# SahakyanLab/GenomeAssembler_dev

Measured on AMD Instinct MI355X. Metric: k-mers built+scored/sec, higher is better.
Workload: dtype u64 keys / u32 counts / f64 scores; 1 GPU; cfg2 (configs[2]): 100 x 50000 bp segments per GPU, 150 bp reads at 50x, k=31, build + breakage scoring of all contigs; mode=segments, segments_total=100, distinct_kmers_rank0=3843627, parallelism=segments sharded over 1 GPU(s), no collective

## Files before the change

### genomeassembler_dev_amd/csrc/kernels.h

```cpp
#pragma once
#include <hip/hip_runtime.h>
#include <stdint.h>

#include "device_utils.h"
#include "keyops.h"

struct ReadSet {
    const u64* words;
    const u64* read_off;
    const u64* seg_read_off;
    const u32* seg_tile_start;
    const uint4* tile_info;
    u32 fixed_len;
    u32 n_segments;
};

__device__ __forceinline__ void read_span(const ReadSet& rs, u64 r, u64* p0, u32* len) {
    if (rs.fixed_len) { *p0 = rs.read_off ? rs.read_off[r] : r * rs.fixed_len; *len = rs.fixed_len; }
    else { const u64 a = rs.read_off[r]; *p0 = a; *len = (u32)(rs.read_off[r + 1] - a); }
}

struct GraphView {
    const void* dk_key;
    const u32* dstart;
// ... 131 lines not shown
template <class K>
__global__ void k_tip_mark(GraphView gv, u32 n_segments, u32 chunks, const u8* eflag, const u32* clen, const u32* nxt, const u32* dk_cnt, const u64* bstart,
                           u32* mult, u32 tip_len, u32* flags, u32* tips);
template <class K>
__global__ void k_bubble_mark(GraphView gv, u32 n_segments, u32 chunks, const u8* eflag, const u32* clen, const u32* nxt, const u32* dk_cnt, const u64* bstart,
                              u32* mult, u32 bubble_len, u32* flags, u32* bubbles);
__global__ void k_kmer_spectrum(const u32* dstart, u32 nb, const u32* dk_cnt, u32 n_segments, u32 chunks, u32* hist);
template <class K>
__global__ void k_lowcov_mark(GraphView gv, u32 n_segments, u32 chunks, const u8* eflag, const u32* clen, const u32* nxt, const u32* dk_cnt, const u64* bstart,
                              u32* mult, u32 cov_len, u32 cov_cutoff, u32* flags, u32* removed);
__global__ void k_contig_cov(const u32* dstart, u32 nb, u32 n_segments, u32 chunks, const u64* link, const u32* e_cid, const u32* dk_cnt,
                             const u32* seg_cstart, unsigned long long* msum, u32* nedges);
template <class K>
__global__ void k_bucket_gather(const K* keys, const u32* mult, const u64* bstart, const u32* dstart, K* dk_key, u32* dk_cnt, u32* claim, u8* eflag,
                                u32* flags);
template <class K> __global__ void k_edge_target(GraphView gv, u32 n_segments, u32 chunks, u32* tgt, u32* claim);
__global__ void k_edge_multi(GraphView gv, u32 n_segments, u32 chunks, const u32* tgt, const u32* claim, u8* eflag);
template <class K>
__global__ void k_node_flags(GraphView gv, u32 n_segments, u32 chunks, const u32* claim, u8* eflag, u64* link, u32* clen);
__global__ void k_edge_next(GraphView gv, u32 n_segments, u32 chunks, const u32* tgt, const u8* eflag, u32* nxt, u64* link);
__global__ void k_link_jump(GraphView gv, u32 n_segments, u32 chunks, u64* link, const u32* prev_active, u32* active, int jumps, const u32* nxt,
                            u32* clen);
__global__ void k_rank_rulers(GraphView gv, u32 n_segments, u32 chunks, u64* link, u32* rtab, u32 rshift, u32* flags);
__global__ void k_rank_lds(GraphView gv, const u32* rtab, u64* link, int max_rounds, u32 rshift, u32 lds_entries, u32* flags);
__global__ void k_chain_len(const u32* nxt, const u64* link, u32* clen, const u32* n_edges_p);
__global__ void k_contig_scan(GraphView gv, const u8* eflag, const u32* clen, u32* e_cid, u64* e_coff, u32* seg_ncontig,
                              u64* seg_cbases, u32* done, u32* seg_cstart, u64* seg_bstart, const u32* flags, u32* report, u32 ticket);
__global__ void k_contig_place(GraphView gv, const u8* eflag, const u32* seg_cstart, const u64* seg_bstart, u32* e_cid, u64* e_coff,
                               u64* c_off, u32 n_segments, u32 chunks);
template <class K>
__global__ void k_contig_emit(GraphView gv, const u64* link, const u32* nxt, const u64* e_coff, u8* out, u32 n_segments, u32 chunks);
__global__ void k_reads_both_strands(const u64* words, const u64* read_off, const u64* seg_read_off, u32 fixed_len, u32 n_segments, u64 n_reads, u32 g,
                                     unsigned long long* out);
template <class K>
__global__ void k_contig_twin(GraphView gv, const u64* link, const u32* e_cid, const u64* c_off, const u32* seg_cstart, const u8* text, u32 n_segments,
                              u32* twin, u32* bad);

template <class K>
__global__ void k_pack_runs(const K* keys, const u32* mult, const u64* bstart, const u32* bucket_d, const u32* gb_list, const u64* dst_off, K* out_keys,
                            u32* out_cnt);
template <class K, int TBL>
__global__ void k_bucket_merge(const K* in_keys, const u32* in_cnt, const u64* run_off, const u32* run_len, u32 n_src, K* out_keys, u32* out_cnt,
                               const u64* bstart, u32* bucket_d, u32* overflow, u16* fdir, int low_bits, const u64* src_base);
__global__ void k_repack_reads(const u64* src, const u64* dir, u64* words_out);
__global__ void k_piece_positions(const u64* piece_first, const u64* piece_word_off, u32 n_pieces, u64 n_reads, u32 fixed_len, u64* pos);
__global__ void k_slice_last(const u32* a, const u64* off, u32 n, u32* out);

__global__ void k_chain_expand(const u64* cwords, const u64* c_off, const u64* sig_off, const u32* elem_contig, const u32* elem_skip, const u64* elem_pos,
                               const u64* out_off, u32 n_scaffolds, u64* out, u64 n_words);
struct ChainSigs {
    const u64* sig_off;
    const u32* elem_contig;
// ... 99 lines not shown
```

### genomeassembler_dev_amd/csrc/kernels_build.hip

```cpp
#include "device_utils.h"
#include "keyops.h"
#include "kernels.h"
#include "dedup_order.h"

typedef unsigned long long u64x2 __attribute__((ext_vector_type(2)));

typedef unsigned int u32x4nt __attribute__((ext_vector_type(4)));
__device__ __forceinline__ uint4 stream_load16(const uint4* p) {
    const u32x4nt v = __builtin_nontemporal_load(reinterpret_cast<const u32x4nt*>(p));
    return make_uint4(v.x, v.y, v.z, v.w);
}
__device__ __forceinline__ void stream_store16(u64x2 v, u64x2* p) { __builtin_nontemporal_store(v, p); }

__global__ void __launch_bounds__(GASM_WG) k_pack_ascii(const u8* __restrict__ ascii, u64 nbases_host, const u64* __restrict__ nbases_dev,
                                                        u64* __restrict__ words, u32* __restrict__ err) {
    const u64 nbases = nbases_dev ? *nbases_dev : nbases_host;
    const u64 nwords = (nbases + 31) / 32 + 4;
    bool ok = true;
    for (u64 t = (u64)blockIdx.x * GASM_WG + threadIdx.x; t < nwords; t += (u64)gridDim.x * GASM_WG) {
        const u64 b0 = t << 5;
        u64 w = 0;
        if (b0 + 32 <= nbases) {
            const uint4* src = reinterpret_cast<const uint4*>(ascii + b0);
            const uint4 v0 = src[0], v1 = src[1];
// ... 123 lines not shown
        for (int d = 1; d < 64; d <<= 1) {
            const u64 o = __shfl_up(inc, d, 64);
            if ((int)ln >= d) inc += o;
        }
        if (ln == 63) s_wave[wv] = inc;
        __syncthreads();
        u64 before = 0, tot = 0;
#pragma unroll
        for (u32 w = 0; w < 16; ++w) { const u64 t = s_wave[w]; if (w < wv) before += t; tot += t; }
        __syncthreads();
        u64 ex = carry + before + inc - sum;
#pragma unroll
        for (u32 q = 0; q < 8; ++q) {
            if (i0 + q < n) out[i0 + q] = (TO)ex;
            ex += v[q];
        }
        carry += tot;
    }
    if (threadIdx.x == 0) out[n] = (TO)carry;
}
template __global__ void k_scan_excl<u64>(const u32*, u64*, u32);
template __global__ void k_scan_excl<u32>(const u32*, u32*, u32);

__device__ __forceinline__ void seg_offsets_wave(const u32* __restrict__ seg_ncontig, const u64* __restrict__ seg_cbases, u32 S,
                                                 u32* __restrict__ seg_cstart, u64* __restrict__ seg_bstart,
                                                 const u32* __restrict__ dstart, u32 nb, const u32* __restrict__ flags,
                                                 u32* __restrict__ report, u32 ticket) {
    const u32 ln = threadIdx.x & 63;
    u32 ccarry = 0;
    u64 bcarry = 0;
    const BuildReport<u32> rep{report, S};
    u32* const rc = &rep.cstart(0);
    u32* const rb = &rep.bstart_lo(0);
    for (u32 base = 0; base < S; base += 64) {
        const u32 i = base + ln;
        const u32 c = i < S ? __hip_atomic_load(&seg_ncontig[i], __ATOMIC_RELAXED, __HIP_MEMORY_SCOPE_AGENT) : 0u;
        const u64 b = i < S ? __hip_atomic_load(&seg_cbases[i], __ATOMIC_RELAXED, __HIP_MEMORY_SCOPE_AGENT) : 0ull;
        const u32 cinc = wave_incl_scan(c);
        u64 binc = b;
#pragma unroll
        for (int d = 1; d < 64; d <<= 1) {
            const u64 o = __shfl_up(binc, d, 64);
            if ((int)ln >= d) binc += o;
        }
        if (i < S) {
            const u32 cs = ccarry + cinc - c;
            const u64 bs = bcarry + binc - b;
            seg_cstart[i] = cs; seg_bstart[i] = bs;
            rc[i] = cs;
            rb[2 * i] = (u32)bs; rb[2 * i + 1] = (u32)(bs >> 32);
            rep.dstart(i) = dstart[(u64)i * nb];
        }
        ccarry += wave_last(cinc);
        bcarry += __shfl(binc, 63, 64);
    }
    if (ln == 0) {
        seg_cstart[S] = ccarry; seg_bstart[S] = bcarry;
        rc[S] = ccarry;
        rb[2 * S] = (u32)bcarry; rb[2 * S + 1] = (u32)(bcarry >> 32);
        rep.dstart(S) = dstart[(u64)S * nb];
        rep.flags() = flags[GASM_FLAG_OVERFLOW];
        rep.rank_failed() = flags[GASM_FLAG_RANK_FAILED];
    }
    __threadfence_system();
    if (ln == 0) rep.ticket() = ticket;
}

template <class K> struct TilePrefetch {
    Roll<K> rl;
    u32 nv, c01, c23, toff, bs_lo, bs_hi;
    template <int N> __device__ __forceinline__ void wait_all_but() {
        rl.template wait_all_but<N>();
        __asm__ volatile("" : "+v"(c01), "+v"(c23), "+v"(toff), "+v"(bs_lo), "+v"(bs_hi));
    }
};

template <class K>
__global__ void __launch_bounds__(GASM_TILE_WG, 1024 / GASM_TILE_WG) k_bucket_scatter(ReadSet rs, const uint4* __restrict__ tinfo, int k, int bbits, u32 g, u32 padm,
                                                                  u32 n_tiles, const u64* __restrict__ bstart, const u32* __restrict__ toff,
                                                                  const ushort4* __restrict__ tcnt, K* __restrict__ keys, u64 scratch) {
    extern __shared__ __align__(16) unsigned char s_raw[];
    constexpr u32 KT = KeyTraits<K>::KT;
    constexpr u32 NFL = KeyTraits<K>::NFL;
    constexpr u32 KPU = TileStage<K>::KPU;
    constexpr u32 CAP = TileStage<K>::CAP;
    const u32 nb = 1u << bbits;
    const u32 tid = threadIdx.x, wv = tid >> 6, ln = tid & 63, sub = tid & 3u;
    const ScatterLds<K> lds{nb};
// ... 809 lines not shown
    const u32 lo = gv.dstart[seg * nb], hi = gv.dstart[(seg + 1) * nb];
    const u32 nr = (hi - lo + rmask) >> rshift;
    for (u32 r = chunk * GASM_WG + threadIdx.x; r < nr; r += chunks * GASM_WG) {
        const u32 i = lo + (r << rshift);
        u32 cur = i, acc = 0, e = GASM_RANK_NONE;
        int step = 0;
        for (; step < 4096; ++step) {
            const u64 l = link[cur];
            if (cur != i) link[cur] = ((u64)i << 32) | GASM_LINK_TAG | acc;
            const u32 a = (u32)(l >> 32);
            if (a == GASM_NONE32) break;
            acc += (u32)l & 0x7FFFFFFFu;
            const u32 al = a - lo;
            if ((l & GASM_LINK_DONE) || !(al & rmask)) { e = (al << 16) | acc; break; }
            if (a == i) break;
            cur = a;
        }
        if (step == 4096) flags[GASM_FLAG_RANK_FAILED] = 1u;
        rtab[(lo >> rshift) + seg + r] = e;
    }
}

#define GASM_RANK_DEAD 0x8000FFFFu
__global__ void __launch_bounds__(1024) k_rank_lds(GraphView gv, const u32* __restrict__ rtab, u64* __restrict__ link, int max_rounds,
                                                    u32 rshift, u32 lds_entries, u32* __restrict__ flags) {
    const u32 rmask = (1u << rshift) - 1u;
    extern __shared__ u32 s_e[];
    __shared__ u32 s_active;
    const u32 seg = blockIdx.x;
    const u32 nb = 1u << gv.bbits;
    const u32 lo = gv.dstart[seg * nb], hi = gv.dstart[(seg + 1) * nb];
    const u32 nr = (hi - lo + rmask) >> rshift;
    if (nr > lds_entries || hi - lo > 65534u) { if (threadIdx.x == 0) flags[GASM_FLAG_RANK_FAILED] = 1u; return; }
    const u32* src = rtab + (lo >> rshift) + seg;
    u32 mine[32];
    u32 live = 0;
#pragma unroll
    for (u32 q = 0; q < 32; ++q) {
        const u32 r = threadIdx.x + 1024 * q;
        u32 e = r < nr ? src[r] : GASM_RANK_NONE;
        bool hopping = false;
        if (e == GASM_RANK_NONE) e = GASM_RANK_DEAD;
        else {
            const u32 a = e >> 16;
            if ((a & rmask) || (a == (r << rshift) && !(e & 0xFFFFu))) e = (0x8000u | r) << 16;
            else if (a == (r << rshift)) e = GASM_RANK_DEAD;
            else { e = ((a >> rshift) << 16) | (e & 0xFFFFu); hopping = true; }
        }
        mine[q] = e;
        if (r < nr) s_e[r] = e;
        live |= (u32)hopping << q;
    }
    for (int round = 0; round < max_rounds; ++round) {
        if (threadIdx.x == 0) s_active = 0;
        __syncthreads();
        u32 any = 0;
#pragma unroll
        for (u32 q0 = 0; q0 < 32; q0 += 8) {
            if (((live >> q0) & 0xFFu) == 0) continue;
            u32 x[8];
#pragma unroll
            for (u32 u = 0; u < 8; ++u) x[u] = s_e[(mine[q0 + u] >> 16) & 0x7FFFu];
#pragma unroll
            for (u32 u = 0; u < 8; ++u) {
                const u32 q = q0 + u;
                const u32 r = threadIdx.x + 1024 * q, e = mine[q];
                const u32 lv = (live >> q) & 1u, stop = x[u] >> 31;
                const u32 hop = lv & ~stop;
                const u32 hopped = (x[u] & 0xFFFF0000u) | ((e + x[u]) & 0xFFFFu);
                const u32 ne = hop ? hopped : e;
                live &= ~((lv & stop) << q);
                any |= hop;
                mine[q] = ne;
                s_e[min(r, nr)] = ne;
            }
        }
        if (any) s_active = 1;
        __syncthreads();
        const bool go = s_active != 0;
        __syncthreads();
        if (!go) break;
    }
#pragma unroll
    for (u32 q = 0; q < 32; ++q) {
        const u32 r = threadIdx.x + 1024 * q;
        if (r >= nr) continue;
        const u32 e = mine[q];
        u64 l = ~0ull;
        if (!((live >> q) & 1u) && e != GASM_RANK_DEAD) {
            const u32 t = (e >> 16) & 0x7FFFu;
            if (s_e[t] != GASM_RANK_DEAD) {
                const u32 ot = src[t];
                l = ((u64)(lo + (ot >> 16)) << 32) | GASM_LINK_DONE | (((e & 0xFFFFu) + (ot & 0xFFFFu)) & 0xFFFFu);
            }
        }
        link[lo + (r << rshift)] = l;
    }
}

__global__ void __launch_bounds__(GASM_WG) k_chain_len(const u32* __restrict__ nxt, const u64* __restrict__ link, u32* __restrict__ clen,
                                                       const u32* __restrict__ n_edges_p) {
    const u32 n_edges = *n_edges_p;
    for (u32 i = blockIdx.x * GASM_WG + threadIdx.x; i < n_edges; i += gridDim.x * GASM_WG) {
        if (nxt[i] != GASM_NONE32) continue;
        const u64 l = link[i];
        const u32 a = (u32)(l >> 32);
        if (a == GASM_NONE32 || !(l & GASM_LINK_DONE)) continue;
        clen[a] = ((u32)l & 0x7FFFFFFFu) + 1;
    }
}

__global__ void __launch_bounds__(1024) k_contig_scan(GraphView gv, const u8* __restrict__ eflag, const u32* __restrict__ clen,
                                                      u32* __restrict__ e_cid, u64* __restrict__ e_coff,
                                                      u32* __restrict__ seg_ncontig, u64* __restrict__ seg_cbases,
                                                      u32* __restrict__ done, u32* __restrict__ seg_cstart, u64* __restrict__ seg_bstart,
                                                      const u32* __restrict__ flags, u32* __restrict__ report, u32 ticket) {
    __shared__ u32 s_last;
    __shared__ u32 s_cnt[16];
    __shared__ u64 s_bas[16];
    const u32 seg = blockIdx.x;
    const u32 nb = 1u << gv.bbits;
    const u32 lo = gv.dstart[seg * nb], hi = gv.dstart[(seg + 1) * nb];
    const u32 wv = threadIdx.x >> 6, ln = threadIdx.x & 63;
    const u32 per = ((hi - lo + 15) / 16 + 63) & ~63u;
    const u32 wa = min(hi, lo + wv * per), wb = min(hi, wa + per);
    u32 ccarry = 0;
    u64 bcarry = 0;
    for (u32 base = wa; base < wb; base += 1024) {
        u32 ef[16];
        u32 cl[16];
#pragma unroll
        for (u32 q = 0; q < 16; ++q) {
            const u32 i = base + q * 64 + ln;
            ef[q] = i < wb ? (u32)eflag[i] : 0u;
            cl[q] = i < wb ? clen[i] : 0u;
        }
#pragma unroll
        for (u32 q = 0; q < 16; ++q) __asm__ volatile("" : "+v"(cl[q]), "+v"(ef[q]));
#pragma unroll
        for (u32 q = 0; q < 16; ++q) {
            const u32 i = base + q * 64 + ln;
            const bool head = ef[q] & 1;
            const u32 len = head ? (u32)(gv.k - 1) + cl[q] : 0u;
            const u32 cinc = wave_incl_scan(head ? 1u : 0u);
            const u32 binc = wave_incl_scan(len);
            if (head) { e_cid[i] = ccarry + cinc - 1; e_coff[i] = bcarry + binc - len; }
            ccarry += wave_last(cinc);
            bcarry += wave_last(binc);
        }
    }
    if (ln == 0) { s_cnt[wv] = ccarry; s_bas[wv] = bcarry; }
    __syncthreads();
    u32 cbefore = 0, ctot = 0;
    u64 bbefore = 0, btot = 0;
#pragma unroll
    for (u32 w = 0; w < 16; ++w) {
        if (w < wv) { cbefore += s_cnt[w]; bbefore += s_bas[w]; }
        ctot += s_cnt[w]; btot += s_bas[w];
    }
    if (wv) {
        for (u32 base = wa + ln; base < wb; base += 2048) {
            u32 ef[32];
#pragma unroll
            for (u32 q = 0; q < 32; ++q) ef[q] = base + 64 * q < wb ? (u32)eflag[base + 64 * q] : 0u;
#pragma unroll
            for (u32 q = 0; q < 32; ++q)
                if (ef[q] & 1) { e_cid[base + 64 * q] += cbefore; e_coff[base + 64 * q] += bbefore; }
        }
    }
    if (threadIdx.x == 0) {
        publish_u32(&seg_ncontig[seg], ctot); publish_u64(&seg_cbases[seg], btot);
        s_last = count_in_last(done) ? 1u : 0u;
    }
    __syncthreads();
    if (!s_last || wv) return;
    seg_offsets_wave(seg_ncontig, seg_cbases, gridDim.x, seg_cstart, seg_bstart, gv.dstart, nb, flags, report, ticket);
}

__global__ void __launch_bounds__(GASM_WG) k_contig_place(GraphView gv, const u8* __restrict__ eflag,
                                                          const u32* __restrict__ seg_cstart, const u64* __restrict__ seg_bstart,
                                                          u32* __restrict__ e_cid, u64* __restrict__ e_coff,
                                                          u64* __restrict__ c_off, u32 n_segments, u32 chunks) {
    if (blockIdx.x == 0 && threadIdx.x == 0) c_off[seg_cstart[n_segments]] = seg_bstart[n_segments];
    for_seg_edges(gv.dstart, 1u << gv.bbits, n_segments, chunks, [&](u32 seg, u32, u32, u32 i) {
        if (!(eflag[i] & 1)) return;
        const u32 cid = seg_cstart[seg] + e_cid[i];
        const u64 off = seg_bstart[seg] + e_coff[i];
        e_cid[i] = cid;
        e_coff[i] = off;
        c_off[cid] = off;
    });
}

__device__ __forceinline__ u32 klow16(u64 a) { return (u32)a & 0xFFFFu; }
__device__ __forceinline__ u32 klow16(const K128& a) { return (u32)a.lo & 0xFFFFu; }
template <class K>
__global__ void __launch_bounds__(GASM_WG) k_contig_emit(GraphView gv, const u64* __restrict__ link, const u32* __restrict__ nxt,
                                                         const u64* __restrict__ e_coff, u8* __restrict__ out, u32 n_segments,
                                                         u32 chunks) {
    for_seg_edge_groups(gv.dstart, 1u << gv.bbits, n_segments, chunks, [&](u32, u32, u32, const u32 (&i)[GASM_EDGE_ILP], const bool (&ok)[GASM_EDGE_ILP]) {
        u64 l[GASM_EDGE_ILP], off[GASM_EDGE_ILP];
        u32 nx[GASM_EDGE_ILP];
        K key[GASM_EDGE_ILP];
        bool on[GASM_EDGE_ILP];
        const int k = gv.k;
        const bool wide = k >= 8;
#pragma unroll
        for (int q = 0; q < GASM_EDGE_ILP; ++q) {
            l[q] = ok[q] ? link[i[q]] : ~0ull;
            nx[q] = ok[q] ? nxt[i[q]] : 0u;
// ... 288 lines not shown
```

### genomeassembler_dev_amd/csrc/pipeline.hip

```cpp
#include <atomic>
#include <chrono>
#include <thread>
#include "pipeline.h"

#include <algorithm>
#include <cmath>

__global__ void k_set_u64(u64* p, u64 v) { *p = v; }

__global__ void k_add_empty_reads(PathSet ps, const u64* __restrict__ seg_empty, u32* __restrict__ poscnt, u32* __restrict__ total) {
    const u32 seg = blockIdx.y;
    const u32 p = ps.seg_path_off[seg] + blockIdx.x * GASM_WG + threadIdx.x;
    if (p >= ps.seg_path_off[seg + 1]) return;
    const u32 e = (u32)seg_empty[seg];
    if (!e) return;
    if (ps.p_off[p + 1] > ps.p_off[p]) poscnt[ps.p_off[p]] += e;
    else total[p] += e;
}

struct Knobs {
    int dedup_tbl = 0, scatter_wgs = 8, hist_wgs = 64, rank_rounds = 18, bbits_add = 0, ruler_shift = 0;
    bool rank_global = false, sync_build = false;
    Knobs() {
        if (const char* v = getenv("GASM_DEDUP_TBL")) dedup_tbl = atoi(v);
// ... 385 lines not shown
                    &d_eflag, &d_nxt, &d_link, &d_clen, &d_ecid, &d_ecoff, &d_rtab, &d_seg_cbases, &d_seg_cstart,
                    &d_seg_bstart, &d_c_off, &d_contig_ascii})
        b->release();
    for (RoundStats& rs : round_stats) rs.d_stats.release();
    part_valid = false;
    if (h_report) { (void)hipHostFree(h_report); h_report = nullptr; h_report_words = 0; }
}

void ScoreState::release() {
    for (DBuf* b : {&d_tbl_off, &d_seed, &d_gpos, &d_poscnt, &d_total, &d_out_f64, &d_out_i32, &d_freq, &d_pd_off, &d_pd, &d_seg_empty, &d_fxsum, &d_first, &d_first_off}) b->release();
}

static int ensure_lds_attrs(gasm_ctx* ctx) {
    if (ctx->lds_attrs_set) return GASM_OK;
#define GASM_LDS_ATTR(kern, bytes) HIPCHK(hipFuncSetAttribute(reinterpret_cast<const void*>(kern), hipFuncAttributeMaxDynamicSharedMemorySize, bytes));
#define GASM_SCORE_LDS_ATTR(T) GASM_LDS_ATTR((k_score_reads_graph<K, T>), GASM_SCORE_PATH_CAP * 12)
    for (int words = 1; words <= 2; ++words)
        GCHK(with_key(words, [&](auto tag) -> int {
            using K = typename decltype(tag)::type;
            GASM_LDS_ATTR(k_bucket_scatter<K>, 160 * 1024) GASM_LDS_ATTR(k_bucket_partition<K>, 160 * 1024) GASM_LDS_ATTR(k_tile_hist<K>, 160 * 1024)
            GASM_SCORE_LDS_ATTR(1) GASM_SCORE_LDS_ATTR(2) GASM_SCORE_LDS_ATTR(3) GASM_SCORE_LDS_ATTR(4) GASM_SCORE_LDS_ATTR(5) GASM_SCORE_LDS_ATTR(6) GASM_SCORE_LDS_ATTR(7) GASM_SCORE_LDS_ATTR(8)
            return GASM_OK;
        }));
    GASM_LDS_ATTR(k_rank_lds, 160 * 1024 - 64)
#undef GASM_SCORE_LDS_ATTR
#undef GASM_LDS_ATTR
    ctx->lds_attrs_set = true;
    return GASM_OK;
}

void distinct_caps(BuildState& bs, u32 S) {
    const u64 limit = bs.multi_pass ? GASM_BUCKET_MAX : bs.small_tbl ? GASM_TBL_LIMIT / 2 : GASM_TBL_LIMIT;
    const u64 per_seg = ((u64)1 << bs.bbits) * limit;
    const u64 all = bs.k < 16 ? ((u64)1 << (2 * bs.k)) : ~(u64)0;
    bs.D_cap = 0; bs.maxD_cap = 0;
    for (u32 s = 0; s < S; ++s) {
        const u64 c = std::min(std::min(bs.h_seg_nk[s], per_seg), all);
        bs.D_cap += c;
        bs.maxD_cap = std::max(bs.maxD_cap, c);
    }
}

static int launch_graph_dense(gasm_ctx* ctx, u32 S, BuildState& bs, bool last_pass);

static GraphView graph_view(const BuildState& bs) {
    GraphView gv;
    gv.dk_key = bs.d_dk_key.p;
    gv.dstart = bs.d_dstart.as<u32>();
    gv.fdir = bs.d_fdir.as<u16>();
    gv.k = bs.k;
    gv.bbits = bs.bbits;
    gv.fbits = bs.fbits;
    return gv;
}

template <class K, int TBL>
static int launch_bucket_dedup_as(gasm_ctx* ctx, BuildState& bs, u32 nbt, const u32* d_blen, u32* d_scan_out) {
    GLAUNCH(ctx, "k_bucket_dedup", (k_bucket_dedup<K, TBL>), dim3(nbt), dim3(GASM_WG), 0, bs.d_keys.as<K>(), bs.d_mult.as<u32>(), bs.d_bstart.as<u64>(), d_blen,
            bs.d_bucket_d.as<u32>(), bs.d_flags.as<u32>(), bs.d_fdir.as<u16>(), 2 * bs.k - bs.bbits, d_scan_out);
    return GASM_OK;
}
static int launch_bucket_dedup(gasm_ctx* ctx, BuildState& bs, u32 nbt, const u32* d_blen, u32* d_scan_out) {
    if (bs.words == 2) return launch_bucket_dedup_as<K128, 2048>(ctx, bs, nbt, d_blen, d_scan_out);
    if (bs.small_tbl) return launch_bucket_dedup_as<u64, 2048>(ctx, bs, nbt, d_blen, d_scan_out);
    return launch_bucket_dedup_as<u64, 4096>(ctx, bs, nbt, d_blen, d_scan_out);
}
// ... 85 lines not shown
        GCHK(bs.d_solid_removed.ensure((size_t)S * 4));
        HIPCHK(hipMemsetAsync(bs.d_solid_removed.p, 0, (size_t)S * 4, ctx->stream));
        GLAUNCH_K(ctx, W, "k_bucket_solid", k_bucket_solid<K>, dim3(nbt), dim3(GASM_WG), 0, bs.d_keys.as<K>(), bs.d_mult.as<u32>(), bs.d_bstart.as<u64>(),
                  bs.d_bucket_d.as<u32>(), bs.d_fdir.as<u16>(), 2 * k - bbits, bs.fbits, bbits, bs.opts.min_count, bs.d_solid_removed.as<u32>(),
                  bs.d_flags.as<u32>() + GASM_FLAG_SOLID_DONE, d_scan_out);
    }
    if (!scan_in_dedup) GLAUNCH(ctx, "k_scan_excl", k_scan_excl<u32>, dim3(1), dim3(1024), 0, bs.d_bucket_d.as<u32>(), bs.d_dstart.as<u32>(), nbt);
    return GASM_OK;
}

static int alloc_graph(BuildState& bs, u32 S) {
    const u64 D = std::max<u64>(bs.D_cap, 1);
    const size_t KB = 8 * (size_t)bs.words;
    if (D >= 0xFFFFFFF0ull) { gasm_set_error("more than 2^32 distinct k-mers possible in one batch: split it"); return GASM_ERR_CAPACITY; }
    GCHK(bs.d_dk_key.ensure(D * KB));
    GCHK(bs.d_dk_cnt.ensure(D * 4));
    GCHK(bs.d_eflag.ensure(D));
    GCHK(bs.d_nxt.ensure(D * 4));
    GCHK(bs.d_link.ensure(D * 8));
    GCHK(bs.d_clen.ensure(D * 4));
    GCHK(bs.d_ecid.ensure(D * 4));
    GCHK(bs.d_ecoff.ensure(D * 8));
    GCHK(bs.d_rtab.ensure((D / 2 + S + 2) * 4));
    GCHK(bs.d_seg_cbases.ensure((size_t)S * 8 + (size_t)S * 4));
    GCHK(bs.d_seg_cstart.ensure(((size_t)S + 1) * 4));
    GCHK(bs.d_seg_bstart.ensure(((size_t)S + 1) * 8));
    bs.bases_cap = D * (u64)bs.k;
    if (bs.bases_cap >= 0xFFFFFFF0ull) { gasm_set_error("contigs could exceed 2^32 bases: split the batch"); return GASM_ERR_CAPACITY; }
    GCHK(bs.d_c_off.ensure((D + 1) * 8));
    GCHK(bs.d_contig_ascii.ensure(bs.bases_cap + 64));
    return GASM_OK;
}

int launch_graph(gasm_ctx* ctx, u32 S, BuildState& bs) {
    const int W = bs.words, bbits = bs.bbits;
    const u32 nb = 1u << bbits, nbt = S * nb;
    GCHK(alloc_graph(bs, S));
    u32* const d_claim = bs.d_nxt.as<u32>();
    const BuildOpts& o = bs.opts;
    const u32 rounds = o.total_rounds();
    for (u32 kind = 0; kind < ROUND_KINDS; ++kind) {
        RoundStats& rs = bs.round_stats[kind];
        if (!o.rounds(kind)) continue;
        GCHK(rs.d_stats.ensure((size_t)2 * rs.max_rounds * S * 4));
        HIPCHK(hipMemsetAsync(rs.d_stats.p, 0, (size_t)2 * rs.max_rounds * S * 4, ctx->stream));
    }
    for (u32 r = 0; r <= rounds; ++r) {
// ... 14 lines not shown
            GLAUNCH_K(ctx, W, "k_tip_mark", k_tip_mark<K>, seg_grid(dchunks, S), dim3(GASM_WG), 0, graph_view(bs), S, dchunks, bs.d_eflag.as<u8>(), bs.d_clen.as<u32>(),
                      bs.d_nxt.as<u32>(), bs.d_dk_cnt.as<u32>(), bs.d_bstart.as<u64>(), bs.d_mult.as<u32>(), o.tip_len, bs.d_flags.as<u32>(), d_contigs);
        } else if (kind == ROUNDS_BUBBLE) {
            GLAUNCH_K(ctx, W, "k_bubble_mark", k_bubble_mark<K>, seg_grid(dchunks, S), dim3(GASM_WG), 0, graph_view(bs), S, dchunks, bs.d_eflag.as<u8>(),
                      bs.d_clen.as<u32>(), bs.d_nxt.as<u32>(), bs.d_dk_cnt.as<u32>(), bs.d_bstart.as<u64>(), bs.d_mult.as<u32>(), o.bubble_len,
                      bs.d_flags.as<u32>(), d_contigs);
        } else {
            GLAUNCH_K(ctx, W, "k_lowcov_mark", k_lowcov_mark<K>, seg_grid(dchunks, S), dim3(GASM_WG), 0, graph_view(bs), S, dchunks, bs.d_eflag.as<u8>(),
                      bs.d_clen.as<u32>(), bs.d_nxt.as<u32>(), bs.d_dk_cnt.as<u32>(), bs.d_bstart.as<u64>(), bs.d_mult.as<u32>(), o.cov_len, o.cov_cutoff,
                      bs.d_flags.as<u32>(), d_contigs);
        }
        u32* const d_scan_out = bs.scan_in_dedup ? bs.d_dstart.as<u32>() : nullptr;
        GLAUNCH_K(ctx, W, "k_bucket_solid", k_bucket_solid<K>, dim3(nbt), dim3(GASM_WG), 0, bs.d_keys.as<K>(), bs.d_mult.as<u32>(), bs.d_bstart.as<u64>(),
                  bs.d_bucket_d.as<u32>(), bs.d_fdir.as<u16>(), 2 * bs.k - bbits, bs.fbits, bbits, 1u, d_kmers, bs.d_flags.as<u32>() + GASM_FLAG_SOLID_DONE, d_scan_out);
        if (!d_scan_out) GLAUNCH(ctx, "k_scan_excl", k_scan_excl<u32>, dim3(1), dim3(1024), 0, bs.d_bucket_d.as<u32>(), bs.d_dstart.as<u32>(), nbt);
    }
    return GASM_OK;
}

static int launch_graph_dense(gasm_ctx* ctx, u32 S, BuildState& bs, bool last_pass) {
    GasmRange range("gasm:graph (degrees, list ranking, contigs)");
    const int W = bs.words;
    u32* const d_claim = bs.d_nxt.as<u32>();
    u32* const d_seg_ncontig = reinterpret_cast<u32*>(bs.d_seg_cbases.as<u64>() + S);
    u32* const d_fl = bs.d_flags.as<u32>();
    const GraphView gv = graph_view(bs);
    const u32 nb = 1u << bs.bbits;
    const u32 est = std::max<u32>(1, (u32)std::min<u64>(bs.maxD_est, bs.maxD_cap));
    const u32 dchunks = (u32)ceil_div_u64(est, GASM_WG);
    const dim3 grid_seg = seg_grid(dchunks, S);
    const u32 gchunks = (u32)ceil_div_u64(est, GASM_WG * GASM_EDGE_ILP);
    const dim3 grid_grp = seg_grid(gchunks, S);
    u32* const d_tgt = bs.d_ecid.as<u32>();
    GLAUNCH_K(ctx, W, "k_edge_target", k_edge_target<K>, grid_seg, dim3(GASM_WG), 0, gv, S, dchunks, d_tgt, d_claim);
    GLAUNCH(ctx, "k_edge_multi", k_edge_multi, grid_grp, dim3(GASM_WG), 0, gv, S, gchunks, d_tgt, d_claim, bs.d_eflag.as<u8>());
    GLAUNCH_K(ctx, W, "k_node_flags", k_node_flags<K>, grid_seg, dim3(GASM_WG), 0, gv, S, dchunks, d_claim, bs.d_eflag.as<u8>(), bs.d_link.as<u64>(), bs.d_clen.as<u32>());
    GLAUNCH(ctx, "k_edge_next", k_edge_next, grid_grp, dim3(GASM_WG), 0, gv, S, gchunks, d_tgt, bs.d_eflag.as<u8>(), bs.d_nxt.as<u32>(), bs.d_link.as<u64>());
    u32* const act = d_fl + GASM_FLAG_ACTIVE;
    const u32 jchunks = (u32)ceil_div_u64(est, GASM_WG * GASM_JUMP_ILP);
    bs.ranked_in_lds = est <= 65534 && !bs.rank_global && !knobs().rank_global;
    bs.ruler_shift = 0;
    if (bs.ranked_in_lds) {
        const u32 rshift = knobs().ruler_shift ? (u32)knobs().ruler_shift : (S >= (u32)ctx->n_cu / 4 ? 1u : 2u);
        bs.ruler_shift = rshift;
        const u32 rchunks = (u32)ceil_div_u64((est + (1u << rshift) - 1) >> rshift, GASM_WG);
        u32 lds_entries = 32767;
        if (S > (u32)ctx->n_cu) lds_entries = std::min<u32>(32767, (((est + est / 4) >> rshift) + 1024) & ~1023u);
        GLAUNCH(ctx, "k_rank_rulers", k_rank_rulers, seg_grid(rchunks, S), dim3(GASM_WG), 0, gv, S, rchunks, bs.d_link.as<u64>(), bs.d_rtab.as<u32>(), rshift, d_fl);
        GLAUNCH(ctx, "k_rank_lds", k_rank_lds, dim3(S), dim3(1024), (size_t)lds_entries * 4 + 4, gv, bs.d_rtab.as<u32>(), bs.d_link.as<u64>(), knobs().rank_rounds, rshift,
                lds_entries, d_fl);
        const int jumps = 255, launches = 2;
        static_assert(launches <= GASM_FLAG_ACTIVE_N, "an active word per launch");
        for (int r = 0; r < launches; ++r)
            GLAUNCH(ctx, "k_link_jump", k_link_jump, seg_grid(jchunks, S), dim3(GASM_WG), 0, gv, S, jchunks, bs.d_link.as<u64>(), r ? act + r - 1 : nullptr, act + r, jumps,
                    bs.d_nxt.as<u32>(), bs.d_clen.as<u32>());
    } else {
        int rounds = 1;
        while ((1ull << rounds) < bs.maxD_cap) ++rounds;
        rounds += 1;
        const int jumps = 4, launches = (rounds * 10 + 22) / 23 + 1;
        if (launches > (int)GASM_FLAG_ACTIVE_N) { gasm_set_error("segment too large for the list-ranking flags"); return GASM_ERR_CAPACITY; }
        for (int r = 0; r < launches; ++r)
            GLAUNCH(ctx, "k_link_jump", k_link_jump, seg_grid(jchunks, S), dim3(GASM_WG), 0, gv, S, jchunks, bs.d_link.as<u64>(), r ? act + r - 1 : nullptr, act + r, jumps,
                    (const u32*)nullptr, (u32*)nullptr);
    }
    const u32 grid_all = (u32)std::min<u64>(ceil_div_u64((u64)est * S, GASM_WG), (u64)ctx->n_cu * 64);
    if (!bs.ranked_in_lds)
        GLAUNCH(ctx, "k_chain_len", k_chain_len, dim3(std::max(1u, grid_all)), dim3(GASM_WG), 0, bs.d_nxt.as<u32>(), bs.d_link.as<u64>(),
                bs.d_clen.as<u32>(), gv.dstart + (size_t)S * nb);
    if (!last_pass) return GASM_OK;
    const size_t words = BuildReport<u32>::words(S);
    if (bs.h_report_words < words) {
        if (bs.h_report) (void)hipHostFree(bs.h_report);
        bs.h_report = nullptr; bs.h_report_words = 0;
        HIPCHK(hipHostMalloc((void**)&bs.h_report, words * 4, hipHostMallocCoherent));
        bs.h_report_words = words;
    }
    bs.ticket = next_ticket();
    BuildReport<volatile u32>{bs.h_report, S}.ticket() = 0;
    GLAUNCH(ctx, "k_contig_scan", k_contig_scan, dim3(S), dim3(1024), 0, gv, bs.d_eflag.as<u8>(), bs.d_clen.as<u32>(),
            bs.d_ecid.as<u32>(), bs.d_ecoff.as<u64>(), d_seg_ncontig, bs.d_seg_cbases.as<u64>(), d_fl + GASM_FLAG_CONTIG_DONE, bs.d_seg_cstart.as<u32>(),
            bs.d_seg_bstart.as<u64>(), d_fl, bs.h_report, bs.ticket);
    GLAUNCH(ctx, "k_contig_place", k_contig_place, grid_seg, dim3(GASM_WG), 0, gv, bs.d_eflag.as<u8>(),
            bs.d_seg_cstart.as<u32>(), bs.d_seg_bstart.as<u64>(), bs.d_ecid.as<u32>(), bs.d_ecoff.as<u64>(), bs.d_c_off.as<u64>(), S, dchunks);
    GLAUNCH_K(ctx, W, "k_contig_emit", k_contig_emit<K>, grid_grp, dim3(GASM_WG), 0, gv, bs.d_link.as<u64>(), bs.d_nxt.as<u32>(),
              bs.d_ecoff.as<u64>(), bs.d_contig_ascii.as<u8>(), S, gchunks);
    bs.pending = true;
    return GASM_OK;
}

int plan_build(gasm_ctx* ctx, DevReads& rd, int k, u64 hint, BuildState& bs) {
    if (k < 2 || k > GASM_MAX_K) { gasm_set_error("k = %d not supported (2..%d)", k, GASM_MAX_K); return GASM_ERR_INVALID; }
    const int W = k <= 31 ? 1 : 2;
    const u32 KT = (u32)with_key(W, [](auto tag) -> int { return KeyTraits<typename decltype(tag)::type>::KT; });
    HIPCHK(hipSetDevice(ctx->device));
    GCHK(ensure_lds_attrs(ctx));
    const u32 S = rd.n_segments;
    const bool same = bs.k == k && bs.words == W && bs.h_seg_nk.size() == S && bs.hint == hint && bs.reads_id == rd.upload_id;
    bs.words = W; bs.k = k; bs.hint = hint; bs.reads_id = rd.upload_id;
    bs.fetched_distinct = bs.fetched_contigs = false;
    bs.pending = false;
    u64 N = 0, maxNs = 0;
    bs.h_seg_nk.assign(S, 0);
    if (rd.fixed_len) {
        const u64 nk = rd.fixed_len >= (u32)k ? rd.fixed_len - k + 1 : 0;
        for (u32 s = 0; s < S; ++s) bs.h_seg_nk[s] = (rd.h_seg_read_off[s + 1] - rd.h_seg_read_off[s]) * nk;
    } else {
// ... 1064 lines not shown
```

Measured before the change: 231.4 billion k-mers/s.

## Split contig scan into per-wave units across workgroups and shrink rank_lds workgroup

The contig prefix scan no longer runs one 1024-thread workgroup per segment. It is spread over several GASM_WG-sized workgroups per segment, each wave publishing a unit count and base sum. A block-wide scan over all units in the last workgroup replaces the per-segment wave scan, and contig_place then applies per-unit offsets, which removes the second fix-up pass over eflag. k_rank_lds moves to 512-thread groups with capped LDS and rereads its entries from LDS instead of keeping a 32-entry register array, so it can sit on a CU beside other kernels. The cost is a larger unit buffer and a serial final scan over S*units entries.

```diff
diff --git a/genomeassembler_dev_amd/csrc/kernels.h b/genomeassembler_dev_amd/csrc/kernels.h
--- a/genomeassembler_dev_amd/csrc/kernels.h
+++ b/genomeassembler_dev_amd/csrc/kernels.h
@@ -177,12 +177,43 @@
 __global__ void k_link_jump(GraphView gv, u32 n_segments, u32 chunks, u64* link, const u32* prev_active, u32* active, int jumps, const u32* nxt,
                             u32* clen);
 __global__ void k_rank_rulers(GraphView gv, u32 n_segments, u32 chunks, u64* link, u32* rtab, u32 rshift, u32* flags);
+#define GASM_CU_LDS (160u * 1024u)
+#define GASM_SCAN_LDS_MAX 1024u
+#define GASM_RANK_WG 512
+#define GASM_RANK_PER_THREAD 32
+#define GASM_RANK_LDS_MAX 65408u
+#define GASM_RANK_ENTRIES_MAX (GASM_RANK_LDS_MAX / 4u - 2u)
+static_assert(GASM_RANK_ENTRIES_MAX <= GASM_RANK_WG * GASM_RANK_PER_THREAD && GASM_RANK_ENTRIES_MAX < 0x8000u, "a thread's entries cover the list; 15-bit ruler indices");
+static_assert(GASM_RANK_LDS_MAX + 4u * 24608u <= GASM_CU_LDS && GASM_RANK_LDS_MAX <= 77648u + 8544u, "k_rank_lds beside four de-duplications / behind one partition workgroup");
+static_assert(GASM_SCAN_LDS_MAX <= 8544u && GASM_SCAN_LDS_MAX <= GASM_CU_LDS - 6u * 24608u, "k_contig_scan beside either streaming kernel");
+constexpr size_t rank_lds_bytes(u32 entries) { return ((size_t)entries + 2) * 4; }
+constexpr u32 rank_lds_entries(u32 est, u32 rshift) {
+    const u64 want = ((((u64)est + est / 4) >> rshift) + 1024) & ~(u64)1023;
+    return (u32)(want < GASM_RANK_ENTRIES_MAX ? want : GASM_RANK_ENTRIES_MAX);
+}
+constexpr u32 rank_fit_shift(u32 est, u32 rshift) {
+    while (rshift < 4 && ((((u64)est + est / 4)) >> rshift) > GASM_RANK_ENTRIES_MAX) ++rshift;
+    return rshift;
+}
+#define GASM_SCAN_ROWS 16
+#define GASM_SCAN_ROUNDS 3
+constexpr u32 scan_units(u32 chunks) { return chunks * (GASM_WG / 64); }
+__host__ __device__ constexpr u32 scan_unit_len(u32 n, u32 units) { return (n / units + (n % units ? 1u : 0u) + 63u) & ~63u; }
+__host__ __device__ constexpr u32 scan_unit_begin(u32 n, u32 units, u32 u) {
+    const u64 a = (u64)u * scan_unit_len(n, units);
+    return a < n ? (u32)a : n;
+}
+constexpr u32 scan_chunks(u32 est, u32 S) {
+    const u32 per_wg = GASM_WG * GASM_SCAN_ROWS * GASM_SCAN_ROUNDS, want = est / per_wg + (est % per_wg ? 1u : 0u), few = S ? 1024u / S : 1024u, cap = few > 16u ? few : 16u;
+    return want < 1u ? 1u : want > cap ? cap : want;
+}
 __global__ void k_rank_lds(GraphView gv, const u32* rtab, u64* link, int max_rounds, u32 rshift, u32 lds_entries, u32* flags);
 __global__ void k_chain_len(const u32* nxt, const u64* link, u32* clen, const u32* n_edges_p);
-__global__ void k_contig_scan(GraphView gv, const u8* eflag, const u32* clen, u32* e_cid, u64* e_coff, u32* seg_ncontig,
-                              u64* seg_cbases, u32* done, u32* seg_cstart, u64* seg_bstart, const u32* flags, u32* report, u32 ticket);
-__global__ void k_contig_place(GraphView gv, const u8* eflag, const u32* seg_cstart, const u64* seg_bstart, u32* e_cid, u64* e_coff,
-                               u64* c_off, u32 n_segments, u32 chunks);
+__global__ void k_contig_scan(GraphView gv, const u8* eflag, const u32* clen, u32* e_cid, u64* e_coff, u32* unit_cnt,
+                              u64* unit_bas, u32 n_segments, u32 chunks, u32* done, u32* seg_cstart, u64* seg_bstart, const u32* flags,
+                              u32* report, u32 ticket);
+__global__ void k_contig_place(GraphView gv, const u8* eflag, const u32* unit_cstart, const u64* unit_bstart, const u32* seg_cstart,
+                               const u64* seg_bstart, u32* e_cid, u64* e_coff, u64* c_off, u32 n_segments, u32 chunks, u32 units);
 template <class K>
 __global__ void k_contig_emit(GraphView gv, const u64* link, const u32* nxt, const u64* e_coff, u8* out, u32 n_segments, u32 chunks);
 __global__ void k_reads_both_strands(const u64* words, const u64* read_off, const u64* seg_read_off, u32 fixed_len, u32 n_segments, u64 n_reads, u32 g,
diff --git a/genomeassembler_dev_amd/csrc/kernels_build.hip b/genomeassembler_dev_amd/csrc/kernels_build.hip
--- a/genomeassembler_dev_amd/csrc/kernels_build.hip
+++ b/genomeassembler_dev_amd/csrc/kernels_build.hip
@@ -169,39 +169,66 @@
 template __global__ void k_scan_excl<u64>(const u32*, u64*, u32);
 template __global__ void k_scan_excl<u32>(const u32*, u32*, u32);
 
-__device__ __forceinline__ void seg_offsets_wave(const u32* __restrict__ seg_ncontig, const u64* __restrict__ seg_cbases, u32 S,
-                                                 u32* __restrict__ seg_cstart, u64* __restrict__ seg_bstart,
-                                                 const u32* __restrict__ dstart, u32 nb, const u32* __restrict__ flags,
-                                                 u32* __restrict__ report, u32 ticket) {
-    const u32 ln = threadIdx.x & 63;
+__device__ __forceinline__ void unit_offsets_block(const u32* __restrict__ unit_cnt, const u64* __restrict__ unit_bas, u32 S, u32 units,
+                                                   u32* __restrict__ unit_cstart, u64* __restrict__ unit_bstart,
+                                                   u32* __restrict__ seg_cstart, u64* __restrict__ seg_bstart,
+                                                   const u32* __restrict__ dstart, u32 nb, const u32* __restrict__ flags,
+                                                   u32* __restrict__ report, u32 ticket, u32* s_cnt, u64* s_bas) {
+    constexpr u32 PER = 8, NW = GASM_WG / 64;
+    const u32 ln = threadIdx.x & 63, wv = threadIdx.x >> 6;
+    const u32 n = S * units;
     u32 ccarry = 0;
     u64 bcarry = 0;
     const BuildReport<u32> rep{report, S};
     u32* const rc = &rep.cstart(0);
     u32* const rb = &rep.bstart_lo(0);
-    for (u32 base = 0; base < S; base += 64) {
-        const u32 i = base + ln;
-        const u32 c = i < S ? __hip_atomic_load(&seg_ncontig[i], __ATOMIC_RELAXED, __HIP_MEMORY_SCOPE_AGENT) : 0u;
-        const u64 b = i < S ? __hip_atomic_load(&seg_cbases[i], __ATOMIC_RELAXED, __HIP_MEMORY_SCOPE_AGENT) : 0ull;
-        const u32 cinc = wave_incl_scan(c);
-        u64 binc = b;
+    for (u32 base = 0; base < n; base += GASM_WG * PER) {
+        const u32 i0 = base + threadIdx.x * PER;
+        u32 c[PER], csum = 0;
+        u64 b[PER], bsum = 0;
+#pragma unroll
+        for (u32 q = 0; q < PER; ++q) {
+            c[q] = i0 + q < n ? __hip_atomic_load(&unit_cnt[i0 + q], __ATOMIC_RELAXED, __HIP_MEMORY_SCOPE_AGENT) : 0u;
+            b[q] = i0 + q < n ? __hip_atomic_load(&unit_bas[i0 + q], __ATOMIC_RELAXED, __HIP_MEMORY_SCOPE_AGENT) : 0ull;
+        }
+#pragma unroll
+        for (u32 q = 0; q < PER; ++q) { csum += c[q]; bsum += b[q]; }
+        const u32 cinc = wave_incl_scan(csum);
+        u64 binc = bsum;
 #pragma unroll
         for (int d = 1; d < 64; d <<= 1) {
             const u64 o = __shfl_up(binc, d, 64);
             if ((int)ln >= d) binc += o;
         }
-        if (i < S) {
-            const u32 cs = ccarry + cinc - c;
-            const u64 bs = bcarry + binc - b;
-            seg_cstart[i] = cs; seg_bstart[i] = bs;
-            rc[i] = cs;
-            rb[2 * i] = (u32)bs; rb[2 * i + 1] = (u32)(bs >> 32);
-            rep.dstart(i) = dstart[(u64)i * nb];
-        }
-        ccarry += wave_last(cinc);
-        bcarry += __shfl(binc, 63, 64);
-    }
-    if (ln == 0) {
+        if (ln == 63) { s_cnt[wv] = cinc; s_bas[wv] = binc; }
+        __syncthreads();
+        u32 cex = ccarry + cinc - csum;
+        u64 bex = bcarry + binc - bsum;
+#pragma unroll
+        for (u32 w = 0; w < NW; ++w) {
+            const u32 ct = s_cnt[w];
+            const u64 bt = s_bas[w];
+            if (w < wv) { cex += ct; bex += bt; }
+            ccarry += ct; bcarry += bt;
+        }
+        __syncthreads();
+        u32 seg = i0 / units, r = i0 - seg * units;
+#pragma unroll
+        for (u32 q = 0; q < PER; ++q) {
+            if (i0 + q < n) {
+                unit_cstart[i0 + q] = cex; unit_bstart[i0 + q] = bex;
+                if (r == 0) {
+                    seg_cstart[seg] = cex; seg_bstart[seg] = bex;
+                    rc[seg] = cex;
+                    rb[2 * seg] = (u32)bex; rb[2 * seg + 1] = (u32)(bex >> 32);
+                    rep.dstart(seg) = dstart[(u64)seg * nb];
+                }
+            }
+            cex += c[q]; bex += b[q];
+            if (++r == units) { r = 0; ++seg; }
+        }
+    }
+    if (threadIdx.x == 0) {
         seg_cstart[S] = ccarry; seg_bstart[S] = bcarry;
         rc[S] = ccarry;
         rb[2 * S] = (u32)bcarry; rb[2 * S + 1] = (u32)(bcarry >> 32);
@@ -210,7 +237,8 @@
         rep.rank_failed() = flags[GASM_FLAG_RANK_FAILED];
     }
     __threadfence_system();
-    if (ln == 0) rep.ticket() = ticket;
+    __syncthreads();
+    if (threadIdx.x == 0) rep.ticket() = ticket;
 }
 
 template <class K> struct TilePrefetch {
@@ -1066,22 +1094,22 @@
 }
 
 #define GASM_RANK_DEAD 0x8000FFFFu
-__global__ void __launch_bounds__(1024) k_rank_lds(GraphView gv, const u32* __restrict__ rtab, u64* __restrict__ link, int max_rounds,
-                                                    u32 rshift, u32 lds_entries, u32* __restrict__ flags) {
+__global__ void __launch_bounds__(GASM_RANK_WG, 8) k_rank_lds(GraphView gv, const u32* __restrict__ rtab, u64* __restrict__ link, int max_rounds,
+                                                                u32 rshift, u32 lds_entries, u32* __restrict__ flags) {
     const u32 rmask = (1u << rshift) - 1u;
     extern __shared__ u32 s_e[];
-    __shared__ u32 s_active;
+    u32& s_active = s_e[lds_entries + 1];
+    constexpr u32 NQ = GASM_RANK_PER_THREAD;
     const u32 seg = blockIdx.x;
     const u32 nb = 1u << gv.bbits;
     const u32 lo = gv.dstart[seg * nb], hi = gv.dstart[(seg + 1) * nb];
     const u32 nr = (hi - lo + rmask) >> rshift;
     if (nr > lds_entries || hi - lo > 65534u) { if (threadIdx.x == 0) flags[GASM_FLAG_RANK_FAILED] = 1u; return; }
     const u32* src = rtab + (lo >> rshift) + seg;
-    u32 mine[32];
     u32 live = 0;
 #pragma unroll
-    for (u32 q = 0; q < 32; ++q) {
-        const u32 r = threadIdx.x + 1024 * q;
+    for (u32 q = 0; q < NQ; ++q) {
+        const u32 r = threadIdx.x + GASM_RANK_WG * q;
         u32 e = r < nr ? src[r] : GASM_RANK_NONE;
         bool hopping = false;
         if (e == GASM_RANK_NONE) e = GASM_RANK_DEAD;
@@ -1091,7 +1119,6 @@
             else if (a == (r << rshift)) e = GASM_RANK_DEAD;
             else { e = ((a >> rshift) << 16) | (e & 0xFFFFu); hopping = true; }
         }
-        mine[q] = e;
         if (r < nr) s_e[r] = e;
         live |= (u32)hopping << q;
     }
@@ -1100,22 +1127,23 @@
         __syncthreads();
         u32 any = 0;
 #pragma unroll
-        for (u32 q0 = 0; q0 < 32; q0 += 8) {
+        for (u32 q0 = 0; q0 < NQ; q0 += 8) {
             if (((live >> q0) & 0xFFu) == 0) continue;
-            u32 x[8];
-#pragma unroll
-            for (u32 u = 0; u < 8; ++u) x[u] = s_e[(mine[q0 + u] >> 16) & 0x7FFFu];
+            u32 own[8], x[8];
+#pragma unroll
+            for (u32 u = 0; u < 8; ++u) own[u] = s_e[min(threadIdx.x + GASM_RANK_WG * (q0 + u), nr)];
+#pragma unroll
+            for (u32 u = 0; u < 8; ++u) x[u] = s_e[(live >> (q0 + u)) & 1u ? (own[u] >> 16) & 0x7FFFu : 0u];
 #pragma unroll
             for (u32 u = 0; u < 8; ++u) {
                 const u32 q = q0 + u;
-                const u32 r = threadIdx.x + 1024 * q, e = mine[q];
+                const u32 r = threadIdx.x + GASM_RANK_WG * q, e = own[u];
                 const u32 lv = (live >> q) & 1u, stop = x[u] >> 31;
                 const u32 hop = lv & ~stop;
                 const u32 hopped = (x[u] & 0xFFFF0000u) | ((e + x[u]) & 0xFFFFu);
                 const u32 ne = hop ? hopped : e;
                 live &= ~((lv & stop) << q);
                 any |= hop;
-                mine[q] = ne;
                 s_e[min(r, nr)] = ne;
             }
         }
@@ -1126,10 +1154,10 @@
         if (!go) break;
     }
 #pragma unroll
-    for (u32 q = 0; q < 32; ++q) {
-        const u32 r = threadIdx.x + 1024 * q;
+    for (u32 q = 0; q < NQ; ++q) {
+        const u32 r = threadIdx.x + GASM_RANK_WG * q;
         if (r >= nr) continue;
-        const u32 e = mine[q];
+        const u32 e = s_e[r];
         u64 l = ~0ull;
         if (!((live >> q) & 1u) && e != GASM_RANK_DEAD) {
             const u32 t = (e >> 16) & 0x7FFFu;
@@ -1154,82 +1182,73 @@
     }
 }
 
-__global__ void __launch_bounds__(1024) k_contig_scan(GraphView gv, const u8* __restrict__ eflag, const u32* __restrict__ clen,
-                                                      u32* __restrict__ e_cid, u64* __restrict__ e_coff,
-                                                      u32* __restrict__ seg_ncontig, u64* __restrict__ seg_cbases,
-                                                      u32* __restrict__ done, u32* __restrict__ seg_cstart, u64* __restrict__ seg_bstart,
-                                                      const u32* __restrict__ flags, u32* __restrict__ report, u32 ticket) {
+__global__ void __launch_bounds__(GASM_WG, 8) k_contig_scan(GraphView gv, const u8* __restrict__ eflag, const u32* __restrict__ clen,
+                                                            u32* __restrict__ e_cid, u64* __restrict__ e_coff,
+                                                            u32* __restrict__ unit_cnt, u64* __restrict__ unit_bas, u32 n_segments, u32 chunks,
+                                                            u32* __restrict__ done, u32* __restrict__ seg_cstart, u64* __restrict__ seg_bstart,
+                                                            const u32* __restrict__ flags, u32* __restrict__ report, u32 ticket) {
     __shared__ u32 s_last;
-    __shared__ u32 s_cnt[16];
-    __shared__ u64 s_bas[16];
-    const u32 seg = blockIdx.x;
+    __shared__ u32 s_cnt[GASM_WG / 64];
+    __shared__ u64 s_bas[GASM_WG / 64];
+    static_assert(sizeof(s_last) + sizeof(s_cnt) + sizeof(s_bas) <= GASM_SCAN_LDS_MAX, "LDS of k_contig_scan");
     const u32 nb = 1u << gv.bbits;
-    const u32 lo = gv.dstart[seg * nb], hi = gv.dstart[(seg + 1) * nb];
     const u32 wv = threadIdx.x >> 6, ln = threadIdx.x & 63;
-    const u32 per = ((hi - lo + 15) / 16 + 63) & ~63u;
-    const u32 wa = min(hi, lo + wv * per), wb = min(hi, wa + per);
-    u32 ccarry = 0;
-    u64 bcarry = 0;
-    for (u32 base = wa; base < wb; base += 1024) {
-        u32 ef[16];
-        u32 cl[16];
-#pragma unroll
-        for (u32 q = 0; q < 16; ++q) {
-            const u32 i = base + q * 64 + ln;
-            ef[q] = i < wb ? (u32)eflag[i] : 0u;
-            cl[q] = i < wb ? clen[i] : 0u;
-        }
-#pragma unroll
-        for (u32 q = 0; q < 16; ++q) __asm__ volatile("" : "+v"(cl[q]), "+v"(ef[q]));
-#pragma unroll
-        for (u32 q = 0; q < 16; ++q) {
-            const u32 i = base + q * 64 + ln;
-            const bool head = ef[q] & 1;
-            const u32 len = head ? (u32)(gv.k - 1) + cl[q] : 0u;
-            const u32 cinc = wave_incl_scan(head ? 1u : 0u);
-            const u32 binc = wave_incl_scan(len);
-            if (head) { e_cid[i] = ccarry + cinc - 1; e_coff[i] = bcarry + binc - len; }
-            ccarry += wave_last(cinc);
-            bcarry += wave_last(binc);
-        }
-    }
-    if (ln == 0) { s_cnt[wv] = ccarry; s_bas[wv] = bcarry; }
+    const u32 units = scan_units(chunks);
+    u32 seg, chunk;
+    if (seg_chunk(n_segments, chunks, &seg, &chunk)) {
+        const u32 lo = gv.dstart[seg * nb], hi = gv.dstart[(seg + 1) * nb];
+        const u32 u = chunk * (GASM_WG / 64) + wv;
+        const u32 wa = lo + scan_unit_begin(hi - lo, units, u), wb = lo + scan_unit_begin(hi - lo, units, u + 1);
+        u32 ccarry = 0;
+        u64 bcarry = 0;
+        for (u32 base = wa; base < wb; base += 64 * GASM_SCAN_ROWS) {
+            u32 ef[GASM_SCAN_ROWS];
+            u32 cl[GASM_SCAN_ROWS];
+#pragma unroll
+            for (u32 q = 0; q < GASM_SCAN_ROWS; ++q) {
+                const u32 i = base + q * 64 + ln;
+                ef[q] = i < wb ? (u32)eflag[i] : 0u;
+                cl[q] = i < wb ? clen[i] : 0u;
+            }
+#pragma unroll
+            for (u32 q = 0; q < GASM_SCAN_ROWS; ++q) __asm__ volatile("" : "+v"(cl[q]), "+v"(ef[q]));
+#pragma unroll
+            for (u32 q = 0; q < GASM_SCAN_ROWS; ++q) {
+                const u32 i = base + q * 64 + ln;
+                const bool head = ef[q] & 1;
+                const u32 len = head ? (u32)(gv.k - 1) + cl[q] : 0u;
+                const u32 cinc = wave_incl_scan(head ? 1u : 0u);
+                const u32 binc = wave_incl_scan(len);
+                if (head) { e_cid[i] = ccarry + cinc - 1; e_coff[i] = bcarry + binc - len; }
+                ccarry += wave_last(cinc);
+                bcarry += wave_last(binc);
+            }
+        }
+        if (ln == 0) {
+            const size_t slot = (size_t)seg * units + u;
+            publish_u32(&unit_cnt[slot], ccarry); publish_u64(&unit_bas[slot], bcarry);
+            __asm__ volatile("s_waitcnt vmcnt(0)" ::: "memory");
+        }
+    }
     __syncthreads();
-    u32 cbefore = 0, ctot = 0;
-    u64 bbefore = 0, btot = 0;
-#pragma unroll
-    for (u32 w = 0; w < 16; ++w) {
-        if (w < wv) { cbefore += s_cnt[w]; bbefore += s_bas[w]; }
-        ctot += s_cnt[w]; btot += s_bas[w];
-    }
-    if (wv) {
-        for (u32 base = wa + ln; base < wb; base += 2048) {
-            u32 ef[32];
-#pragma unroll
-            for (u32 q = 0; q < 32; ++q) ef[q] = base + 64 * q < wb ? (u32)eflag[base + 64 * q] : 0u;
-#pragma unroll
-            for (u32 q = 0; q < 32; ++q)
-                if (ef[q] & 1) { e_cid[base + 64 * q] += cbefore; e_coff[base + 64 * q] += bbefore; }
-        }
-    }
-    if (threadIdx.x == 0) {
-        publish_u32(&seg_ncontig[seg], ctot); publish_u64(&seg_cbases[seg], btot);
-        s_last = count_in_last(done) ? 1u : 0u;
-    }
+    if (threadIdx.x == 0) s_last = count_in_last(done) ? 1u : 0u;
     __syncthreads();
-    if (!s_last || wv) return;
-    seg_offsets_wave(seg_ncontig, seg_cbases, gridDim.x, seg_cstart, seg_bstart, gv.dstart, nb, flags, report, ticket);
+    if (!s_last) return;
+    unit_offsets_block(unit_cnt, unit_bas, n_segments, units, unit_cnt + (size_t)n_segments * units, unit_bas + (size_t)n_segments * units,
+                       seg_cstart, seg_bstart, gv.dstart, nb, flags, report, ticket, s_cnt, s_bas);
 }
 
 __global__ void __launch_bounds__(GASM_WG) k_contig_place(GraphView gv, const u8* __restrict__ eflag,
+                                                          const u32* __restrict__ unit_cstart, const u64* __restrict__ unit_bstart,
                                                           const u32* __restrict__ seg_cstart, const u64* __restrict__ seg_bstart,
                                                           u32* __restrict__ e_cid, u64* __restrict__ e_coff,
-                                                          u64* __restrict__ c_off, u32 n_segments, u32 chunks) {
+                                                          u64* __restrict__ c_off, u32 n_segments, u32 chunks, u32 units) {
     if (blockIdx.x == 0 && threadIdx.x == 0) c_off[seg_cstart[n_segments]] = seg_bstart[n_segments];
-    for_seg_edges(gv.dstart, 1u << gv.bbits, n_segments, chunks, [&](u32 seg, u32, u32, u32 i) {
+    for_seg_edges(gv.dstart, 1u << gv.bbits, n_segments, chunks, [&](u32 seg, u32 lo, u32 hi, u32 i) {
         if (!(eflag[i] & 1)) return;
-        const u32 cid = seg_cstart[seg] + e_cid[i];
-        const u64 off = seg_bstart[seg] + e_coff[i];
+        const size_t slot = (size_t)seg * units + (i - lo) / scan_unit_len(hi - lo, units);
+        const u32 cid = unit_cstart[slot] + e_cid[i];
+        const u64 off = unit_bstart[slot] + e_coff[i];
         e_cid[i] = cid;
         e_coff[i] = off;
         c_off[cid] = off;
diff --git a/genomeassembler_dev_amd/csrc/pipeline.hip b/genomeassembler_dev_amd/csrc/pipeline.hip
--- a/genomeassembler_dev_amd/csrc/pipeline.hip
+++ b/genomeassembler_dev_amd/csrc/pipeline.hip
@@ -431,7 +431,7 @@
             GASM_SCORE_LDS_ATTR(1) GASM_SCORE_LDS_ATTR(2) GASM_SCORE_LDS_ATTR(3) GASM_SCORE_LDS_ATTR(4) GASM_SCORE_LDS_ATTR(5) GASM_SCORE_LDS_ATTR(6) GASM_SCORE_LDS_ATTR(7) GASM_SCORE_LDS_ATTR(8)
             return GASM_OK;
         }));
-    GASM_LDS_ATTR(k_rank_lds, 160 * 1024 - 64)
+    GASM_LDS_ATTR(k_rank_lds, GASM_RANK_LDS_MAX)
 #undef GASM_SCORE_LDS_ATTR
 #undef GASM_LDS_ATTR
     ctx->lds_attrs_set = true;
@@ -451,6 +451,7 @@
 }
 
 static int launch_graph_dense(gasm_ctx* ctx, u32 S, BuildState& bs, bool last_pass);
+static u32 graph_est(const BuildState& bs) { return std::max<u32>(1, (u32)std::min<u64>(bs.maxD_est, bs.maxD_cap)); }
 
 static GraphView graph_view(const BuildState& bs) {
     GraphView gv;
@@ -582,7 +583,7 @@
     GCHK(bs.d_ecid.ensure(D * 4));
     GCHK(bs.d_ecoff.ensure(D * 8));
     GCHK(bs.d_rtab.ensure((D / 2 + S + 2) * 4));
-    GCHK(bs.d_seg_cbases.ensure((size_t)S * 8 + (size_t)S * 4));
+    GCHK(bs.d_seg_cbases.ensure((size_t)S * scan_units(scan_chunks(graph_est(bs), S)) * 24));
     GCHK(bs.d_seg_cstart.ensure(((size_t)S + 1) * 4));
     GCHK(bs.d_seg_bstart.ensure(((size_t)S + 1) * 8));
     bs.bases_cap = D * (u64)bs.k;
@@ -643,11 +644,10 @@
     GasmRange range("gasm:graph (degrees, list ranking, contigs)");
     const int W = bs.words;
     u32* const d_claim = bs.d_nxt.as<u32>();
-    u32* const d_seg_ncontig = reinterpret_cast<u32*>(bs.d_seg_cbases.as<u64>() + S);
     u32* const d_fl = bs.d_flags.as<u32>();
     const GraphView gv = graph_view(bs);
     const u32 nb = 1u << bs.bbits;
-    const u32 est = std::max<u32>(1, (u32)std::min<u64>(bs.maxD_est, bs.maxD_cap));
+    const u32 est = graph_est(bs);
     const u32 dchunks = (u32)ceil_div_u64(est, GASM_WG);
     const dim3 grid_seg = seg_grid(dchunks, S);
     const u32 gchunks = (u32)ceil_div_u64(est, GASM_WG * GASM_EDGE_ILP);
@@ -662,13 +662,12 @@
     bs.ranked_in_lds = est <= 65534 && !bs.rank_global && !knobs().rank_global;
     bs.ruler_shift = 0;
     if (bs.ranked_in_lds) {
-        const u32 rshift = knobs().ruler_shift ? (u32)knobs().ruler_shift : (S >= (u32)ctx->n_cu / 4 ? 1u : 2u);
+        const u32 rshift = knobs().ruler_shift ? (u32)knobs().ruler_shift : rank_fit_shift(est, S >= (u32)ctx->n_cu / 4 ? 1u : 2u);
         bs.ruler_shift = rshift;
         const u32 rchunks = (u32)ceil_div_u64((est + (1u << rshift) - 1) >> rshift, GASM_WG);
-        u32 lds_entries = 32767;
-        if (S > (u32)ctx->n_cu) lds_entries = std::min<u32>(32767, (((est + est / 4) >> rshift) + 1024) & ~1023u);
+        const u32 lds_entries = S > (u32)ctx->n_cu ? rank_lds_entries(est, rshift) : GASM_RANK_ENTRIES_MAX;
         GLAUNCH(ctx, "k_rank_rulers", k_rank_rulers, seg_grid(rchunks, S), dim3(GASM_WG), 0, gv, S, rchunks, bs.d_link.as<u64>(), bs.d_rtab.as<u32>(), rshift, d_fl);
-        GLAUNCH(ctx, "k_rank_lds", k_rank_lds, dim3(S), dim3(1024), (size_t)lds_entries * 4 + 4, gv, bs.d_rtab.as<u32>(), bs.d_link.as<u64>(), knobs().rank_rounds, rshift,
+        GLAUNCH(ctx, "k_rank_lds", k_rank_lds, dim3(S), dim3(GASM_RANK_WG), rank_lds_bytes(lds_entries), gv, bs.d_rtab.as<u32>(), bs.d_link.as<u64>(), knobs().rank_rounds, rshift,
                 lds_entries, d_fl);
         const int jumps = 255, launches = 2;
         static_assert(launches <= GASM_FLAG_ACTIVE_N, "an active word per launch");
@@ -699,11 +698,15 @@
     }
     bs.ticket = next_ticket();
     BuildReport<volatile u32>{bs.h_report, S}.ticket() = 0;
-    GLAUNCH(ctx, "k_contig_scan", k_contig_scan, dim3(S), dim3(1024), 0, gv, bs.d_eflag.as<u8>(), bs.d_clen.as<u32>(),
-            bs.d_ecid.as<u32>(), bs.d_ecoff.as<u64>(), d_seg_ncontig, bs.d_seg_cbases.as<u64>(), d_fl + GASM_FLAG_CONTIG_DONE, bs.d_seg_cstart.as<u32>(),
+    const u32 schunks = scan_chunks(est, S), units = scan_units(schunks);
+    const size_t n_units = (size_t)S * units;
+    u64* const d_unit_bas = bs.d_seg_cbases.as<u64>();
+    u32* const d_unit_cnt = reinterpret_cast<u32*>(d_unit_bas + 2 * n_units);
+    GLAUNCH(ctx, "k_contig_scan", k_contig_scan, seg_grid(schunks, S), dim3(GASM_WG), 0, gv, bs.d_eflag.as<u8>(), bs.d_clen.as<u32>(),
+            bs.d_ecid.as<u32>(), bs.d_ecoff.as<u64>(), d_unit_cnt, d_unit_bas, S, schunks, d_fl + GASM_FLAG_CONTIG_DONE, bs.d_seg_cstart.as<u32>(),
             bs.d_seg_bstart.as<u64>(), d_fl, bs.h_report, bs.ticket);
-    GLAUNCH(ctx, "k_contig_place", k_contig_place, grid_seg, dim3(GASM_WG), 0, gv, bs.d_eflag.as<u8>(),
-            bs.d_seg_cstart.as<u32>(), bs.d_seg_bstart.as<u64>(), bs.d_ecid.as<u32>(), bs.d_ecoff.as<u64>(), bs.d_c_off.as<u64>(), S, dchunks);
+    GLAUNCH(ctx, "k_contig_place", k_contig_place, grid_seg, dim3(GASM_WG), 0, gv, bs.d_eflag.as<u8>(), d_unit_cnt + n_units, d_unit_bas + n_units,
+            bs.d_seg_cstart.as<u32>(), bs.d_seg_bstart.as<u64>(), bs.d_ecid.as<u32>(), bs.d_ecoff.as<u64>(), bs.d_c_off.as<u64>(), S, dchunks, units);
     GLAUNCH_K(ctx, W, "k_contig_emit", k_contig_emit<K>, grid_grp, dim3(GASM_WG), 0, gv, bs.d_link.as<u64>(), bs.d_nxt.as<u32>(),
               bs.d_ecoff.as<u64>(), bs.d_contig_ascii.as<u8>(), S, gchunks);
     bs.pending = true;
```

Measured after the change: 232.8 billion k-mers/s (median of 6 runs). No clear change (+0.6%).
